# dog-qiuqiu/Yolo-FastestV2

Measured on AMD Instinct MI355X. Metric: images/sec at 352x352 bs=256 per GPU (forward+decode+NMS), higher is better.
Workload: dtype f32 tensors; contractions fp16x3 (two-term fp16 split operands on v_mfma_f32_16x16x32_f16, fp32 accumulate); depthwise/BN/ReLU/decode/NMS fp32 VALU; 1 GPU

## Files before the change

### include/yfv2.h

```cpp
#ifndef YFV2_H
#define YFV2_H

#include <stdint.h>

#ifdef __cplusplus
extern "C" {
#endif

#define YFV2_ABI_VERSION 7
#define YFV2_API __attribute__((visibility("default")))
#define YFV2_MAX_DET 300

typedef enum yfv2_status {
  YFV2_OK = 0,
  YFV2_ERR_ARG = -1,
  YFV2_ERR_CONFIG = -2,
  YFV2_ERR_DEVICE = -3,
  YFV2_ERR_WEIGHTS = -4,
  YFV2_ERR_STATE = -5,
  YFV2_ERR_BATCH = -6,
  YFV2_ERR_RANGE = -7
} yfv2_status;

typedef struct yfv2_ctx* yfv2_handle;
// ... 302 lines not shown
YFV2_API int32_t yfv2_num_rows(yfv2_handle h);
YFV2_API int32_t yfv2_num_stages(yfv2_handle h);

YFV2_API int yfv2_stage_info(yfv2_handle h, int32_t i, char* name, int32_t name_cap, double* flops_per_image,
                    double* bytes_per_image, double* external_bytes_per_image);
YFV2_API int yfv2_stage_kernel(yfv2_handle h, int32_t i, char* name, int32_t name_cap);

YFV2_API int yfv2_profile_forward(yfv2_handle h, const float* x, int32_t B, float* const out6[6], int32_t iters,
                         float* ms, void* stream);

YFV2_API int yfv2_clock_probe_begin(yfv2_handle h, int32_t workgroups, float milliseconds, int32_t busy, void* stream);
YFV2_API int yfv2_clock_probe_end(yfv2_handle h, double out[6], void* stream);

YFV2_API int yfv2_debug_repeat_step(yfv2_handle h, const float* x, int32_t B, float* const out6[6], int32_t step, int32_t iters, void* stream);

YFV2_API int yfv2_debug_post(yfv2_handle h, const float* const out6[6], int32_t B, float conf_thres, double iou_thres,
                             float* dets, int32_t* idx, int32_t* count, void* stream);

YFV2_API int64_t yfv2_debug_activation(yfv2_handle h, int32_t which, int32_t B, float* host_dst, int64_t cap);

YFV2_API int64_t yfv2_debug_train_relu_output(yfv2_handle h, const char* conv_name, float* host_dst, int64_t capacity);
YFV2_API int64_t yfv2_debug_train_tensor(yfv2_handle h, const char* name, int32_t which, float* host_dst, int64_t capacity);

YFV2_API int yfv2_debug_plan_dryrun(const yfv2_config* cfg, const yfv2_tensor_desc* tensors, int32_t n, int32_t* n_steps, int64_t* blob_floats);
YFV2_API int yfv2_debug_plan_dryrun_ex(const yfv2_config* cfg, const yfv2_plan* plan, const yfv2_tensor_desc* tensors, int32_t n, int32_t* n_steps,
                                       int64_t* blob_floats);
YFV2_API int64_t yfv2_debug_plan_image(const yfv2_config* cfg, const yfv2_tensor_desc* tensors, int32_t n, int32_t step, char* name,
                                       int32_t name_cap, float* dst, int64_t cap);
YFV2_API int64_t yfv2_debug_plan_image_ex(const yfv2_config* cfg, const yfv2_plan* plan, const yfv2_tensor_desc* tensors, int32_t n, int32_t step,
                                          char* name, int32_t name_cap, float* dst, int64_t cap);
YFV2_API int yfv2_debug_plan_c2_label(const yfv2_config* cfg, const yfv2_tensor_desc* tensors, int32_t n, int32_t* label);
YFV2_API int yfv2_debug_rows(int32_t row_kind, int32_t yuv, int32_t w, int32_t W, int64_t* lds_bytes, int32_t* max_width);
YFV2_API int yfv2_debug_rows16(int32_t row_kind, int32_t w, int32_t W, int64_t* lds_bytes, int32_t* max_width);

#ifdef __cplusplus
}
#endif
#endif
```

### yolo_fastestv2_amd/_lib.py

```python
import ctypes as C
import os

_HERE = os.path.dirname(os.path.abspath(__file__))
LIB_PATH = os.environ.get("YFV2_LIB") or os.path.join(_HERE, "libyfv2.so")
ABI_VERSION = 7
MAX_DET = 300

OK, ERR_ARG, ERR_CONFIG, ERR_DEVICE, ERR_WEIGHTS, ERR_STATE, ERR_BATCH, ERR_RANGE = 0, -1, -2, -3, -4, -5, -6, -7


class Config(C.Structure):
    _fields_ = [("classes", C.c_int32), ("anchor_num", C.c_int32), ("height", C.c_int32), ("width", C.c_int32),
                ("anchors", C.c_double * 12), ("max_batch", C.c_int32), ("device", C.c_int32)]


class Plan(C.Structure):
    _fields_ = [("struct_size", C.c_int32), ("fp32_matrix", C.c_int32), ("layer_by_layer", C.c_int32), ("post_two_launches", C.c_int32),
                ("front_two_launches", C.c_int32), ("towers_unpaired", C.c_int32), ("lanes", C.c_int32), ("trace", C.c_int32), ("trace_step", C.c_int32)]


PLAN_FIELDS = ("fp32_matrix", "layer_by_layer", "post_two_launches", "front_two_launches", "towers_unpaired", "lanes", "trace", "trace_step")


def make_plan(plan=None):
# ... 162 lines not shown
    "yfv2_track_update_motion": (C.c_int, [C.c_void_p, C.c_void_p, C.c_void_p, C.c_int32, C.c_int32, C.POINTER(C.c_int32), C.c_void_p, C.c_int32,
                                           C.POINTER(TrackRule), C.POINTER(TrackMotion), C.c_void_p, C.c_void_p, C.c_void_p, C.c_void_p, C.c_void_p,
                                           C.c_void_p, C.c_void_p]),
    "yfv2_track_update_two_pass": (C.c_int, [C.c_void_p, C.c_void_p, C.c_void_p, C.c_int32, C.c_int32, C.POINTER(C.c_int32), C.c_void_p, C.c_int32,
                                             C.POINTER(TrackRule), C.POINTER(TrackMotion), C.POINTER(TrackSecond), C.c_void_p, C.c_void_p, C.c_void_p,
                                             C.c_void_p, C.c_void_p, C.c_void_p, C.c_void_p, C.c_void_p]),
    "yfv2_track_feature_words": (C.c_int64, [C.c_int32, C.c_int32]),
    "yfv2_track_cosine": (C.c_int, [C.POINTER(C.c_float), C.POINTER(C.c_float), C.c_int32, C.POINTER(C.c_float), C.POINTER(C.c_float)]),
    "yfv2_track_feature_step": (C.c_int, [C.POINTER(C.c_float), C.c_int32, C.POINTER(C.c_float), C.c_int32, C.c_float, C.POINTER(C.c_float),
                                          C.POINTER(C.c_int32)]),
    "yfv2_track_update_appearance": (C.c_int, [C.c_void_p, C.c_void_p, C.c_void_p, C.c_int32, C.c_int32, C.POINTER(C.c_int32), C.c_void_p, C.c_int32,
                                               C.POINTER(TrackRule), C.POINTER(TrackMotion), C.POINTER(TrackSecond), C.POINTER(TrackAppearance),
                                               C.c_void_p, C.c_void_p, C.c_void_p, C.c_void_p, C.c_void_p, C.c_void_p, C.c_void_p, C.c_void_p,
                                               C.c_void_p, C.c_void_p, C.c_void_p]),
    "yfv2_export_maps": (C.c_int, [C.c_void_p, C.POINTER(C.c_void_p), C.c_int32, C.c_void_p, C.c_void_p, C.c_void_p]),
    "yfv2_deploy_post": (C.c_int, [C.c_void_p, C.c_void_p, C.c_void_p, C.c_int32, C.c_void_p, C.c_float, C.c_float, C.c_void_p, C.c_void_p,
                                   C.c_int32, C.c_void_p]),
    "yfv2_deploy_dropped": (C.c_int, [C.c_void_p, C.POINTER(C.c_int32), C.c_void_p]),
    "yfv2_detect_deploy_frames_u8": (C.c_int, [C.c_void_p, C.POINTER(Frame), C.c_int32, C.c_float, C.c_float, C.c_void_p, C.c_void_p,
                                               C.c_int32, C.c_void_p]),
    "yfv2_anchor_kmeans": (C.c_int, [C.c_void_p, C.c_void_p, C.c_int64, C.c_void_p, C.c_int32, C.c_int32, C.c_void_p, C.c_void_p,
                                     C.POINTER(KmeansInfo), C.c_void_p]),
    "yfv2_debug_kmeans_group": (C.c_int, [C.c_void_p, C.c_int32]),
    "yfv2_ap_per_class": (C.c_int, [C.c_void_p, C.c_void_p, C.c_void_p, C.c_void_p, C.c_int64, C.c_void_p, C.c_int64, C.POINTER(ApResult), C.c_void_p]),
    "yfv2_ap_per_class_multi": (C.c_int, [C.c_void_p, C.c_void_p, C.c_void_p, C.c_void_p, C.c_int64, C.c_void_p, C.c_int64, C.c_int32,
                                          C.POINTER(ApResult), C.c_void_p]),
    "yfv2_debug_plan_dryrun": (C.c_int, [C.c_void_p, C.c_void_p, C.c_int32, C.POINTER(C.c_int32), C.POINTER(C.c_int64)]),
    "yfv2_debug_plan_dryrun_ex": (C.c_int, [C.c_void_p, C.POINTER(Plan), C.c_void_p, C.c_int32, C.POINTER(C.c_int32), C.POINTER(C.c_int64)]),
    "yfv2_debug_plan_image": (C.c_int64, [C.c_void_p, C.c_void_p, C.c_int32, C.c_int32, C.c_char_p, C.c_int32, C.c_void_p, C.c_int64]),
    "yfv2_debug_plan_image_ex": (C.c_int64, [C.c_void_p, C.POINTER(Plan), C.c_void_p, C.c_int32, C.c_int32, C.c_char_p, C.c_int32, C.c_void_p, C.c_int64]),
    "yfv2_debug_plan_c2_label": (C.c_int, [C.c_void_p, C.c_void_p, C.c_int32, C.POINTER(C.c_int32)]),
    "yfv2_debug_rows": (C.c_int, [C.c_int32, C.c_int32, C.c_int32, C.c_int32, C.POINTER(C.c_int64), C.POINTER(C.c_int32)]),
    "yfv2_debug_rows16": (C.c_int, [C.c_int32, C.c_int32, C.c_int32, C.POINTER(C.c_int64), C.POINTER(C.c_int32)]),
    "yfv2_num_rows": (C.c_int32, [C.c_void_p]),
    "yfv2_num_stages": (C.c_int32, [C.c_void_p]),
    "yfv2_stage_info": (C.c_int, [C.c_void_p, C.c_int32, C.c_char_p, C.c_int32, C.POINTER(C.c_double),
                                  C.POINTER(C.c_double), C.POINTER(C.c_double)]),
    "yfv2_stage_kernel": (C.c_int, [C.c_void_p, C.c_int32, C.c_char_p, C.c_int32]),
    "yfv2_profile_forward": (C.c_int, [C.c_void_p, C.c_void_p, C.c_int32, C.POINTER(C.c_void_p), C.c_int32,
                                       C.POINTER(C.c_float), C.c_void_p]),
    "yfv2_debug_repeat_step": (C.c_int, [C.c_void_p, C.c_void_p, C.c_int32, C.POINTER(C.c_void_p), C.c_int32, C.c_int32, C.c_void_p]),
    "yfv2_debug_post": (C.c_int, [C.c_void_p, C.POINTER(C.c_void_p), C.c_int32, C.c_float, C.c_double, C.c_void_p, C.c_void_p,
                                  C.c_void_p, C.c_void_p]),
    "yfv2_debug_activation": (C.c_int64, [C.c_void_p, C.c_int32, C.c_int32, C.c_void_p, C.c_int64]),
    "yfv2_debug_train_relu_output": (C.c_int64, [C.c_void_p, C.c_char_p, C.c_void_p, C.c_int64]),
    "yfv2_debug_train_tensor": (C.c_int64, [C.c_void_p, C.c_char_p, C.c_int32, C.c_void_p, C.c_int64]),
}

_lib = None


def lib():
    global _lib
    if _lib is not None:
        return _lib
    if not os.path.exists(LIB_PATH):
        raise ImportError("%s is missing: the HIP extension has not been built (run __graft_entry__.build()); "
                          "yolo_fastestv2_amd has no CPU or PyTorch fallback" % LIB_PATH)
    L = C.CDLL(LIB_PATH)
    if not hasattr(L, "yfv2_abi_version"):
        raise ImportError("%s does not export yfv2_abi_version: not a libyfv2 build" % LIB_PATH)
    L.yfv2_abi_version.restype, L.yfv2_abi_version.argtypes = C.c_int, []
    if L.yfv2_abi_version() != ABI_VERSION:
        raise ImportError("libyfv2.so ABI %d != binding ABI %d: rebuild (__graft_entry__.build())" % (L.yfv2_abi_version(), ABI_VERSION))
    for name, (res, args) in _PROTOTYPES.items():
        if name.startswith("yfv2_debug_") and os.environ.get("YFV2_LIB") and not hasattr(L, name):
# ... 17 lines not shown
```

### yolo_fastestv2_amd/csrc/yfv2_api_debug.hip

```cpp
#include <algorithm>
#include <cstdio>
#include <variant>

#include "yfv2_ctx.h"

namespace {

struct DryRun {
  yfv2_ctx ctx;
  WeightPacker wp;
  int build(const yfv2_config* cfg, const yfv2_plan* plan, const yfv2_tensor_desc* tensors, int32_t n) {
    int rows = 0;
    if (int rc = check_config(cfg, &rows)) return rc;
    uintptr_t next = 0x100000000ull;
    auto fake = [&](yfv2_ctx* hh, Buf* b, size_t per_img) {
      b->per_img = per_img;
      b->p = reinterpret_cast<float*>(next);
      next += (per_img * sizeof(float) * (size_t)hh->cfg.max_batch + 4095) & ~(uintptr_t)4095;
      return (int)YFV2_OK;
    };
    setup_ctx(&ctx, cfg, rows, fake);
    read_plan_switches(&ctx, plan);
    return build_plan(&ctx, wp, tensors, n, nullptr);
  }
// ... 41 lines not shown
  const size_t img = job >= 0 ? tw->halves[job].img : step_image(view[step]);
  if (name && name_cap > 0) std::snprintf(name, (size_t)name_cap, "%s", st_name.c_str());
  const int64_t avail = (int64_t)d.wp.blob.size() - (int64_t)img;
  const int64_t cnt = avail < cap ? avail : cap;
  if (cnt > 0) std::memcpy(dst, &d.wp.blob[img], sizeof(float) * (size_t)cnt);
  return cnt;
}

int yfv2_debug_plan_c2_label(const yfv2_config* cfg, const yfv2_tensor_desc* tensors, int32_t n, int32_t* label) {
  if (!cfg || !tensors || n <= 0 || !label) return fail(nullptr, YFV2_ERR_ARG, "yfv2_debug_plan_c2_label: bad argument");
  DryRun d;
  if (int rc = d.build(cfg, nullptr, tensors, n)) return rc;
  for (int k = 0; k < 96; ++k) label[k] = d.ctx.plan.c2_permuted ? d.ctx.plan.c2_label[k] : k;
  return d.ctx.plan.c2_permuted ? 1 : 0;
}

int yfv2_debug_rows(int32_t row_kind, int32_t yuv, int32_t w, int32_t W, int64_t* lds_bytes, int32_t* max_width) {
  if (row_kind < 0 || row_kind >= YFV2_ROW_KINDS || yuv < 0 || yuv > 1 || w < 1 || w > (1 << 26) || W < 1 || W > (1 << 20))
    return fail(nullptr, YFV2_ERR_ARG, "yfv2_debug_rows: bad argument");
  const Yfv2FrameKind frames = yuv ? YFV2_FRAMES_YUV8 : YFV2_FRAMES_BGR;
  if (lds_bytes) *lds_bytes = (int64_t)yfv2_rows_lds_bytes((Yfv2RowKind)row_kind, frames, w, W);
  if (max_width) *max_width = yfv2_rows_max_width((Yfv2RowKind)row_kind, frames, W);
  return YFV2_OK;
}

int yfv2_debug_rows16(int32_t row_kind, int32_t w, int32_t W, int64_t* lds_bytes, int32_t* max_width) {
  if (row_kind < 0 || row_kind >= YFV2_ROW_KINDS || w < 1 || w > (1 << 26) || W < 1 || W > (1 << 20))
    return fail(nullptr, YFV2_ERR_ARG, "yfv2_debug_rows16: bad argument");
  if (lds_bytes) *lds_bytes = (int64_t)yfv2_rows_lds_bytes((Yfv2RowKind)row_kind, YFV2_FRAMES_YUV16, w, W);
  if (max_width) *max_width = yfv2_rows_max_width((Yfv2RowKind)row_kind, YFV2_FRAMES_YUV16, W);
  return YFV2_OK;
}

int yfv2_clock_probe_begin(yfv2_handle h, int32_t workgroups, float milliseconds, int32_t busy, void* stream) {
  if (!h || workgroups < 1 || workgroups > 4096 || !(milliseconds > 0.f) || milliseconds > 10000.f)
    return fail(h, YFV2_ERR_ARG, "yfv2_clock_probe_begin: bad argument");
  DeviceGuard guard(h->device);
  if (!h->d_probe) HIP_TRY(h, hipMalloc(reinterpret_cast<void**>(&h->d_probe), 4096 * 4 * sizeof(unsigned long long)));
  int khz = 0;
  if (hipDeviceGetAttribute(&khz, hipDeviceAttributeWallClockRate, h->device) != hipSuccess || khz <= 0) khz = 100000;
  ClockProbeArgs a{};
  a.out = h->d_probe; a.busy = busy ? 1 : 0;
  a.ref_ticks = (unsigned long long)((double)milliseconds * (double)khz);
  h->probe_wgs = workgroups;
  if (!yfv2_launch_clock_probe(a, workgroups, static_cast<hipStream_t>(stream))) return fail(h, YFV2_ERR_DEVICE, "clock probe launch failed");
  return YFV2_OK;
}

int yfv2_clock_probe_end(yfv2_handle h, double out[6], void* stream) {
  if (!h || !out) return fail(h, YFV2_ERR_ARG, "yfv2_clock_probe_end: null argument");
  if (!h->d_probe || h->probe_wgs < 1) return fail(h, YFV2_ERR_STATE, "yfv2_clock_probe_end without yfv2_clock_probe_begin");
  DeviceGuard guard(h->device);
  hipStream_t s = static_cast<hipStream_t>(stream);
  std::vector<unsigned long long> st((size_t)h->probe_wgs * 4);
  HIP_TRY(h, hipMemcpyAsync(st.data(), h->d_probe, st.size() * sizeof(unsigned long long), hipMemcpyDeviceToHost, s));
  HIP_TRY(h, hipStreamSynchronize(s));
  int khz = 0;
  if (hipDeviceGetAttribute(&khz, hipDeviceAttributeWallClockRate, h->device) != hipSuccess || khz <= 0) khz = 100000;
  const double ref_mhz = khz * 1e-3;
  double mn = 1e30, mx = 0., sum = 0., ms = 0.;
  unsigned xcds = 0;
  for (int i = 0; i < h->probe_wgs; ++i) {
    const double cyc = (double)st[4 * i], ref = (double)st[4 * i + 1];
    if (!(ref > 0.)) return fail(h, YFV2_ERR_DEVICE, "clock probe: a workgroup reported no reference ticks");
    const double mhz = cyc / ref * ref_mhz;
    mn = std::min(mn, mhz); mx = std::max(mx, mhz); sum += mhz; ms += ref / ref_mhz * 1e-3;
// ... 155 lines not shown
```

### yolo_fastestv2_amd/csrc/yfv2_block.hip

```cpp
#include <cstdlib>
#include <type_traits>

#include "yfv2_device.h"

template <int C2>
struct S1Cfg {
  static constexpr int KC = (C2 + 15) / 16;
  static constexpr int DW_FL = 9 * KC * 16;
  static constexpr int CST_FL = 6 * KC * 16;
};

constexpr int CH_TBL_FL = 64;

constexpr int CH6_WP_FL = 3 * 3 * 256;
constexpr int CH6_IMG_FL = 2 * CH6_WP_FL + S1Cfg<48>::DW_FL + S1Cfg<48>::CST_FL + CH_TBL_FL;

__host__ __device__ constexpr int s1chain_pitch(int PW) { return 2 * (PW + 1) + ((PW - 2 * (PW + 1)) % 16 + 16) % 16; }
__host__ __device__ constexpr int s1chain_plane(int PH, int PW) { return (2 * (PH + 1) * s1chain_pitch(PW) + 15) & ~15; }

template <int THREADS>
__global__ __launch_bounds__(THREADS, 2) void block_s1chain6_kernel(BlockS1Args a) {
  constexpr int C2 = 48;
  using Cfg = S1Cfg<C2>;
  constexpr int KC = Cfg::KC, NQ = C2 / 4, C = 2 * C2, NT = 4;
  constexpr int NW = THREADS / 64;
  constexpr int N4 = CH6_IMG_FL / 4, NIT = (N4 + THREADS - 1) / THREADS;
  extern __shared__ __attribute__((aligned(16))) float lds[];
  float* IM = lds;
  float* T1 = lds + CH6_IMG_FL;
  const float* W1P = IM;
  const float* W2P = IM + CH6_WP_FL;
  const float* WD = IM + 2 * CH6_WP_FL;
  const float* CS = WD + Cfg::DW_FL;
  const int H = a.H, W = a.W, HW = H * W, NB = a.nblk;
// ... 322 lines not shown
  const long pl = s1chain_plane(H / 2, W / 2);
  return (long)CH6_IMG_FL + 12L * pl * 4;
}

long yfv2_s1chain_park_floats(int H, int W, int nblk) { return 12L * (nblk - 2) * ((((H / 2) * (W / 2) + 15) & ~15) * 4); }

int yfv2_s1chain_image_floats() { return CH6_IMG_FL; }

bool yfv2_s1chain_supported(int c2, int H, int W) {
  if (c2 != 48 || H < 2 || (H & 1) || (W & 1)) return false;
  if ((H / 2) * (W / 2) > 16 * 8) return false;
  if (yfv2_s1chain_park_floats(H, W, 7) > 24L * (4 * H) * (4 * W)) return false;
  return s1chain_lds_floats(H, W) * 4 <= YFV2_LDS_FULL;
}

bool yfv2_launch_block_s1chain(const BlockS1Args& a, hipStream_t s) {
  if (!yfv2_s1chain_supported(48, a.H, a.W) || a.nblk < 2) return false;
  const size_t lds = sizeof(float) * (size_t)s1chain_lds_floats(a.H, a.W);
  const Yfv2Device dev = yfv2_device();
  YFV2_LAUNCH_LDS(dev, (block_s1chain6_kernel<512>), YFV2_LDS_FULL, dim3(yfv2_image_grid(a.B, dev)), dim3(512), lds, s, a);
  return true;
}

constexpr int P96_C2 = 96, P96_C = 192, P96_KC = 6, P96_TH = 3, P96_TC = 32;
constexpr int P96_CPP = P96_C + 4;
constexpr int P96_TP = P96_TC + 4;
constexpr int P96_W1_FL = 2 * P96_KC * 256, P96_W2_FL = P96_KC * 2 * 256;
constexpr int P96_IMG_FL = P96_W1_FL + P96_W2_FL + 9 * P96_TC + 4 * P96_TC + 2 * P96_C2;
constexpr int P96_W1P_FL = 2 * (P96_KC / 2) * 2 * 256, P96_W2P_FL = P96_KC * 1 * 2 * 256;
constexpr int P96_IMGP_FL = P96_W1P_FL + P96_W2P_FL + 9 * P96_TC + 4 * P96_TC + 2 * P96_C2;
constexpr int P96_MAXPX = 128;

template <int THREADS, bool PRE>
__global__ __launch_bounds__(THREADS, 2) void block_s1pool_kernel(BlockS1Args a) {
  constexpr int NW = THREADS / 64;
  constexpr int IMG_FL = PRE ? P96_IMGP_FL : P96_IMG_FL;
  constexpr int W1_FL = PRE ? P96_W1P_FL : P96_W1_FL, W2_FL = PRE ? P96_W2P_FL : P96_W2_FL;
  constexpr int N4 = IMG_FL / 4, NIT = (N4 + THREADS - 1) / THREADS;
  extern __shared__ __attribute__((aligned(16))) float lds[];
  float* POOL = lds;
  float* T = POOL + a.H * a.W * P96_CPP;
  float* IMG = T + (a.H + 2) * (a.W + 2) * P96_TP;
  Yfv2Watch watch;
  const int H = a.H, W = a.W, HW = H * W, WP = W + 2, NB = a.nblk;
  const float invW = 1.0f / (float)W;
  const int tid = threadIdx.x, lane = tid & 63, p = lane & 15, g = lane >> 4, wave = tid >> 6;
  const int px = 16 * wave + p;
  const bool pv = px < HW;
  const int pxc = pv ? px : HW - 1;
  const int py = yfv2_fdiv(pxc, invW), pxx = pxc - py * W;
  float* tpix = T + ((py + 1) * WP + pxx + 1) * P96_TP;
  const float* twin = T + (py * WP + pxx) * P96_TP;
  float* ppix = POOL + pxc * P96_CPP;
  static_assert(NW * 16 >= P96_MAXPX, "one tile per wave");

  YFV2_WSTAMP(0);
  for (int i = tid; i < (H + 2) * WP * P96_TP / 4; i += THREADS) reinterpret_cast<f32x4*>(T)[i] = (f32x4){0.f, 0.f, 0.f, 0.f};

  for (int b = blockIdx.x; b < a.B; b += gridDim.x) {
    {
      const f32x4* src = reinterpret_cast<const f32x4*>(a.in + (size_t)b * HW * P96_C);
      const f32x4* isrc = reinterpret_cast<const f32x4*>(a.img);
      constexpr int NPX = (P96_MAXPX * (P96_C / 4) + THREADS - 1) / THREADS;
      const int n4 = HW * (P96_C / 4);
      f32x4 ti[NIT];
#pragma unroll
      for (int k = 0; k < NIT; ++k) { const int i = tid + k * THREADS; ti[k] = i < N4 ? isrc[i] : (f32x4){0.f, 0.f, 0.f, 0.f}; }
#pragma unroll
      for (int k0 = 0; k0 < NPX; k0 += 6) {
        f32x4 tp[6];
#pragma unroll
        for (int k = 0; k < 6; ++k) { const int i = tid + (k0 + k) * THREADS; tp[k] = i < n4 ? src[i] : (f32x4){0.f, 0.f, 0.f, 0.f}; }
#pragma unroll
        for (int k = 0; k < 6; ++k) {
          const int i = tid + (k0 + k) * THREADS;
          const int ipx = i / (P96_C / 4), q = i - ipx * (P96_C / 4);
          if (i < n4) *reinterpret_cast<f32x4*>(POOL + ipx * P96_CPP + 4 * q) = tp[k];
        }
      }
#pragma unroll
      for (int k = 0; k < NIT; ++k) { const int i = tid + k * THREADS; if (i < N4) reinterpret_cast<f32x4*>(IMG)[i] = ti[k]; }
    }
    __syncthreads();
    YFV2_WSTAMP(1);

#pragma unroll 1
    for (int blk = 0; blk < NB; ++blk) {
      f32x4 acc2[P96_KC];
#pragma unroll
      for (int mt = 0; mt < P96_KC; ++mt) acc2[mt] = (f32x4){0.f, 0.f, 0.f, 0.f};
      yfv2_h8 b1a[PRE ? P96_KC / 2 : 1], b1b[PRE ? P96_KC / 2 : 1];
      auto split_pair = [&](f32x4 c0, f32x4 c1, yfv2_h8& t1, yfv2_h8& t2) __attribute__((always_inline)) {
        u32x4 u1, u2;
        const f32x4 cs[2] = {c0 * 16.0f, c1 * 16.0f};
#pragma unroll
        for (int e = 0; e < 2; ++e) {
          const u32x4 t = split_f16x2(cs[e]);
          u1[2 * e] = t[0]; u1[2 * e + 1] = t[1]; u2[2 * e] = t[2]; u2[2 * e + 1] = t[3];
        }
        t1 = __builtin_bit_cast(yfv2_h8, u1); t2 = __builtin_bit_cast(yfv2_h8, u2);
      };
      if constexpr (PRE) {
#pragma unroll
        for (int sp = 0; sp < P96_KC / 2; ++sp) {
          f32x4 c[2];
#pragma unroll
          for (int e = 0; e < 2; ++e) {
            const int s2 = 2 * sp + e;
            const f32x4 q0 = *reinterpret_cast<const f32x4*>(ppix + 32 * s2 + 8 * g);
            const f32x4 q1 = *reinterpret_cast<const f32x4*>(ppix + 32 * s2 + 8 * g + 4);
            c[e] = (f32x4){q0[1], q0[3], q1[1], q1[3]};
          }
          split_pair(c[0], c[1], b1a[sp], b1b[sp]);
        }
      }
#pragma unroll 1
      for (int th = 0; th < P96_TH; ++th) {
        const int t = blk * P96_TH + th;
        const bool more = t + 1 < NB * P96_TH;
        const float* W1t = IMG;
        const float* W2t = IMG + W1_FL;
        const float* TAPS = W2t + W2_FL;
        const float* CSV = TAPS + 9 * P96_TC;
        f32x4 nimg[NIT];
        {
          const f32x4* isrc = reinterpret_cast<const f32x4*>(a.img + (size_t)(t + 1) * IMG_FL);
#pragma unroll
          for (int k = 0; k < NIT; ++k) { const int i = tid + k * THREADS; nimg[k] = (more && i < N4) ? isrc[i] : (f32x4){0.f, 0.f, 0.f, 0.f}; }
        }
        {
          f32x4 acc1[2] = {{0.f, 0.f, 0.f, 0.f}, {0.f, 0.f, 0.f, 0.f}};
          if constexpr (PRE) {
#pragma unroll
            for (int sp = 0; sp < P96_KC / 2; ++sp) {
              yfv2_h8 a1[2], a2[2];
#pragma unroll
              for (int mt = 0; mt < 2; ++mt) {
                const float* wq2 = W1t + (((mt * (P96_KC / 2) + sp) * 2) * 64 + lane) * 4;
                a1[mt] = __builtin_bit_cast(yfv2_h8, *reinterpret_cast<const u32x4*>(wq2));
                a2[mt] = __builtin_bit_cast(yfv2_h8, *reinterpret_cast<const u32x4*>(wq2 + 256));
              }
#define P96_PROD(A_, B_) _Pragma("unroll") for (int mt = 0; mt < 2; ++mt) acc1[mt] = __builtin_amdgcn_mfma_f32_16x16x32_f16(A_[mt], B_, acc1[mt], 0, 0, 0);
              P96_PROD(a1, b1b[sp]) P96_PROD(a2, b1a[sp]) P96_PROD(a1, b1a[sp])
#undef P96_PROD
            }
            watch.see(acc1[0][0]);
          } else {
#pragma unroll
          for (int s2 = 0; s2 < P96_KC; ++s2) {
            const f32x4 q0 = *reinterpret_cast<const f32x4*>(ppix + 32 * s2 + 8 * g);
            const f32x4 q1 = *reinterpret_cast<const f32x4*>(ppix + 32 * s2 + 8 * g + 4);
            const f32x4 bf = {q0[1], q0[3], q1[1], q1[3]};
            const f32x4 a0 = *reinterpret_cast<const f32x4*>(W1t + ((0 * P96_KC + s2) * 64 + lane) * 4);
            const f32x4 a1 = *reinterpret_cast<const f32x4*>(W1t + ((1 * P96_KC + s2) * 64 + lane) * 4);
#pragma unroll
            for (int j = 0; j < 4; ++j) {
              acc1[0] = __builtin_amdgcn_mfma_f32_16x16x4f32(a0[j], bf[j], acc1[0], 0, 0, 0);
              acc1[1] = __builtin_amdgcn_mfma_f32_16x16x4f32(a1[j], bf[j], acc1[1], 0, 0, 0);
            }
          }
          }
          if (pv) {
#pragma unroll
            for (int mt = 0; mt < 2; ++mt) {
              const f32x4 sc = *reinterpret_cast<const f32x4*>(CSV + 0 * P96_TC + 16 * mt + 4 * g);
              const f32x4 sh = *reinterpret_cast<const f32x4*>(CSV + 1 * P96_TC + 16 * mt + 4 * g);
              f32x4 y;
#pragma unroll
              for (int c = 0; c < 4; ++c) { const float u = __builtin_fmaf(acc1[mt][c], sc[c], sh[c]); y[c] = u > 0.f ? u : 0.f; }
              *reinterpret_cast<f32x4*>(tpix + 16 * mt + 4 * g) = y;
            }
          }
        }
        if (blk == 0) YFV2_WSTAMP(2 + 4 * th);
        __syncthreads();
        if (blk == 0) YFV2_WSTAMP(3 + 4 * th);
        if constexpr (PRE) {
          f32x4 bfr2[2];
#pragma unroll
          for (int c2 = 0; c2 < 2; ++c2) {
            const int cb = 16 * c2 + 4 * g;
            f32x4 win[9], wl[9];
#pragma unroll
            for (int k = 0; k < 9; ++k) {
              win[k] = *reinterpret_cast<const f32x4*>(twin + ((k / 3) * WP + (k % 3)) * P96_TP + cb);
// ... 19 lines not shown
            a2[mt] = __builtin_bit_cast(yfv2_h8, *reinterpret_cast<const u32x4*>(wq2 + 256));
          }
#define P96_PROD(A_, B_) _Pragma("unroll") for (int mt = 0; mt < P96_KC; ++mt) acc2[mt] = __builtin_amdgcn_mfma_f32_16x16x32_f16(A_[mt], B_, acc2[mt], 0, 0, 0);
          P96_PROD(a1, x2) P96_PROD(a2, x1) P96_PROD(a1, x1)
#undef P96_PROD
        } else {
#pragma unroll
        for (int c2 = 0; c2 < 2; ++c2) {
          const int cb = 16 * c2 + 4 * g;
          f32x4 win[9], wl[9], af[P96_KC];
#pragma unroll
          for (int k = 0; k < 9; ++k) {
            win[k] = *reinterpret_cast<const f32x4*>(twin + ((k / 3) * WP + (k % 3)) * P96_TP + cb);
            wl[k] = *reinterpret_cast<const f32x4*>(TAPS + k * P96_TC + cb);
          }
          const f32x4 dsc = *reinterpret_cast<const f32x4*>(CSV + 2 * P96_TC + cb);
          const f32x4 dsh = *reinterpret_cast<const f32x4*>(CSV + 3 * P96_TC + cb);
#pragma unroll
          for (int mt = 0; mt < P96_KC; ++mt) af[mt] = *reinterpret_cast<const f32x4*>(W2t + ((mt * 2 + c2) * 64 + lane) * 4);
          __builtin_amdgcn_sched_barrier(0);
          f32x4 d = {0.f, 0.f, 0.f, 0.f}, bfr;
#pragma unroll
          for (int k = 0; k < 9; ++k)
#pragma unroll
            for (int c = 0; c < 4; ++c) d[c] = __builtin_fmaf(win[k][c], wl[k][c], d[c]);
#pragma unroll
          for (int c = 0; c < 4; ++c) bfr[c] = __builtin_fmaf(d[c], dsc[c], dsh[c]);
#pragma unroll
          for (int j = 0; j < 4; ++j)
#pragma unroll
            for (int mt = 0; mt < P96_KC; ++mt) acc2[mt] = __builtin_amdgcn_mfma_f32_16x16x4f32(af[mt][j], bfr[j], acc2[mt], 0, 0, 0);
        }
        }
        if (th == P96_TH - 1) {
          if constexpr (PRE) watch.see(acc2[0][0]);
#pragma unroll
          for (int mt = 0; mt < P96_KC; ++mt) {
            const f32x4 sc = *reinterpret_cast<const f32x4*>(CSV + 4 * P96_TC + 16 * mt + 4 * g);
            const f32x4 sh = *reinterpret_cast<const f32x4*>(CSV + 4 * P96_TC + P96_C2 + 16 * mt + 4 * g);
#pragma unroll
            for (int c = 0; c < 4; ++c) { const float u = __builtin_fmaf(acc2[mt][c], sc[c], sh[c]); acc2[mt][c] = u > 0.f ? u : 0.f; }
          }
        }
        if (blk == 0) YFV2_WSTAMP(4 + 4 * th);
        __syncthreads();
        if (more) {
#pragma unroll
          for (int k = 0; k < NIT; ++k) { const int i = tid + k * THREADS; if (i < N4) reinterpret_cast<f32x4*>(IMG)[i] = nimg[k]; }
        }
        if (th < P96_TH - 1) __syncthreads();
        if (blk == 0) YFV2_WSTAMP(5 + 4 * th);
      }
      {
        constexpr int NQ = P96_C2 / 4;
        constexpr int NEV = (P96_MAXPX * NQ + THREADS - 1) / THREADS;
        f32x4 ev[NEV];
#pragma unroll
        for (int k = 0; k < NEV; ++k) {
          const int i = tid + k * THREADS;
          const int ipx = i / NQ, q = i - ipx * NQ;
          ev[k] = (f32x4){0.f, 0.f, 0.f, 0.f};
          if (ipx < HW) {
            const f32x4 q0 = *reinterpret_cast<const f32x4*>(POOL + ipx * P96_CPP + 8 * q);
            const f32x4 q1 = *reinterpret_cast<const f32x4*>(POOL + ipx * P96_CPP + 8 * q + 4);
            ev[k] = (f32x4){q0[0], q0[2], q1[0], q1[2]};
          }
        }
        __syncthreads();
#pragma unroll
        for (int k = 0; k < NEV; ++k) {
          const int i = tid + k * THREADS;
          const int ipx = i / NQ, q = i - ipx * NQ;
          if (ipx < HW) *reinterpret_cast<f32x4*>(POOL + ipx * P96_CPP + 4 * q) = ev[k];
        }
        if (pv) {
#pragma unroll
          for (int mt = 0; mt < P96_KC; ++mt) *reinterpret_cast<f32x4*>(ppix + P96_C2 + 16 * mt + 4 * g) = acc2[mt];
        }
        __syncthreads();
        YFV2_WSTAMP(14 + blk);
      }
    }
    {
      f32x4* dst = reinterpret_cast<f32x4*>(a.out + (size_t)b * HW * P96_C);
      for (int i = tid; i < HW * (P96_C / 4); i += THREADS) {
        const int ipx = i / (P96_C / 4), q = i - ipx * (P96_C / 4);
        dst[i] = *reinterpret_cast<const f32x4*>(POOL + ipx * P96_CPP + 4 * q);
      }
    }
    YFV2_WSTAMP(17);
    __syncthreads();
  }
  watch.report(a.nonfinite);
}

static long s1pool_lds_floats(int H, int W, bool pre) { return (long)H * W * P96_CPP + (long)(H + 2) * (W + 2) * P96_TP + (pre ? P96_IMGP_FL : P96_IMG_FL); }
int yfv2_s1pool_image_floats(bool presplit) { return presplit ? P96_IMGP_FL : P96_IMG_FL; }
bool yfv2_s1pool_supported(int c2, int H, int W) {
  if (c2 != P96_C2 || H * W > P96_MAXPX || H * W < 1) return false;
  return s1pool_lds_floats(H, W, true) * 4 <= YFV2_LDS_FULL;
}

bool yfv2_launch_block_s1pool(const BlockS1Args& a, hipStream_t s) {
  if (!yfv2_s1pool_supported(P96_C2, a.H, a.W) || a.nblk < 1) return false;
  const size_t lds = sizeof(float) * (size_t)s1pool_lds_floats(a.H, a.W, a.presplit != 0);
  const Yfv2Device dev = yfv2_device();
  const int blocks = yfv2_image_grid(a.B, dev);
  if (a.presplit) YFV2_LAUNCH_LDS(dev, (block_s1pool_kernel<512, true>), YFV2_LDS_FULL, dim3(blocks), dim3(512), lds, s, a);
  else YFV2_LAUNCH_LDS(dev, (block_s1pool_kernel<512, false>), YFV2_LDS_FULL, dim3(blocks), dim3(512), lds, s, a);
  return true;
}

constexpr int TW_C = 72, TW_KC = 5;
constexpr int TW_WP_FL = TW_KC * TW_KC * 256;
constexpr int TW_WH_FL = TW_KC * 256;

template <int CIN>
struct S2Cfg {
  static constexpr int KC = (CIN + 15) / 16;
  static constexpr int CP = CIN + 4;
  static constexpr int W_FL = KC * KC * 256;
  static constexpr int DW_FL = 9 * KC * 16;
  static constexpr int NCS = 10;
  static constexpr int MAXP = 14;
  static constexpr int MAXT = CIN <= 24 ? 10 : 6;
};

template <int CIN, int THREADS, bool PPIN>
__global__ __launch_bounds__(THREADS) void block_s2_kernel(BlockS2Args a) {
  using Cfg = S2Cfg<CIN>;
  constexpr int KC = Cfg::KC, CP = Cfg::CP, KS = KC * 16;
  constexpr int NW = THREADS / 64;
  constexpr int CO = 2 * CIN;
  extern __shared__ __attribute__((aligned(16))) float lds[];
  float* W1 = lds;
  float* W2 = W1 + Cfg::W_FL;
  float* WJ = W2 + Cfg::W_FL;
  float* WD = WJ + Cfg::W_FL;
  float* WE = WD + Cfg::DW_FL;
  float* CS = WE + Cfg::DW_FL;
  float* T1 = CS + Cfg::NCS * KS;
  const int H = a.H, W = a.W, R = a.R, OH = H >> 1, OW = W >> 1;
// ... 894 lines not shown
```

### yolo_fastestv2_amd/csrc/yfv2_internal.h

```cpp
#pragma once
#include <hip/hip_runtime.h>
#include <hip/hip_ext.h>
#include <stdint.h>

#include <atomic>

struct Yfv2LaunchProbe { hipEvent_t start = nullptr, stop = nullptr; int launches = 0; };
extern thread_local Yfv2LaunchProbe yfv2_launch_probe;
#define YFV2_LAUNCH(kernel, grid, block, lds, stream, ...)                                                                        \
  do {                                                                                                                             \
    Yfv2LaunchProbe& yfv2_lp_ = yfv2_launch_probe;                                                                                 \
    hipExtLaunchKernelGGL(kernel, grid, block, lds, stream, yfv2_lp_.launches++ == 0 ? yfv2_lp_.start : nullptr, yfv2_lp_.stop, 0, \
                          __VA_ARGS__);                                                                                            \
  } while (0)
struct Yfv2Device { int index, cus; };
inline Yfv2Device yfv2_device() {
  static std::atomic<int> cus_of[64];
  int dev = 0;
  if (hipGetDevice(&dev) != hipSuccess || dev < 0 || dev > 63) dev = 0;
  int cus = cus_of[dev].load(std::memory_order_relaxed);
  if (cus <= 0) { if (hipDeviceGetAttribute(&cus, hipDeviceAttributeMultiprocessorCount, dev) != hipSuccess || cus <= 0) cus = 256; cus_of[dev].store(cus, std::memory_order_relaxed); }
  return {dev, cus};
}
inline int yfv2_device_cus() { return yfv2_device().cus; }
// ... 56 lines not shown
struct DwArgs {
  const float* in;
  float* out;
  const float* w;
  const float* scale;
  const float* shift;
  int B, H, W, C;
  int OH, OW;
  int in_stride, in_off;
  int out_stride, out_off;
  int relu;
};

struct BlockS1Args {
  const float* in;
  float* out;
  const float* img;
  long long* trace;
  int B, H, W;
  int R;
  int nblk;
  int presplit;
  int* nonfinite;
  float* park;
};

bool yfv2_s1chain_supported(int c2, int H, int W);
int yfv2_s1chain_image_floats();
long yfv2_s1chain_park_floats(int H, int W, int nblk);
bool yfv2_launch_block_s1chain(const BlockS1Args& a, hipStream_t s);
bool yfv2_s1pool_supported(int c2, int H, int W);
int yfv2_s1pool_image_floats(bool presplit);
bool yfv2_launch_block_s1pool(const BlockS1Args& a, hipStream_t s);

struct BlockS2Args {
  const float* in;
  float* out;
  const float* img;
  int B, H, W;
  int R;
  int s4_main_bands;
  int pp_in;
  unsigned pp_mask;
  long long pp_bufstride;
  long long pp_imgstride;
  int bf6;
  long long* trace;
  const float* img16;
  int* nonfinite;
};
bool yfv2_s3h_supported(int H, int W);
void yfv2_launch_s3h(const BlockS2Args& a, hipStream_t s);
bool yfv2_s4h_supported(int H, int W);
void yfv2_launch_s4h(const BlockS2Args& a, hipStream_t s);

__host__ __device__ inline int yfv2_stage2_channel(int slot) {
  const int p = slot >> 1, e = slot & 1;
  const int b0 = p / 12, b1 = (p % 12) / 6, b2 = (p % 6) / 3, h = 2 * (p % 3) + e;
  return b0 + 2 * b1 + 4 * b2 + 8 * h;
}
struct S1PxArgs {
  float* act;
  const float* img;
  int B, H, W;
  int nstrips, nb, R;
  int img_stride;
// ... 419 lines not shown
```

Measured before the change: 478,200 images/s.

## Replace per-block channel shuffle in s1pool kernel with host-planned LDS slot tables

Precomputes, on the host, a channel-to-LDS-slot assignment for the stride-1 ShuffleNet block chain so the channel shuffle between blocks becomes pure addressing. The in-kernel gather/scatter pass that repacked even channels after every block, along with its two barriers, is removed. Loads, stores and operand reads now go through small byte tables passed as a kernel argument and copied into LDS. The next-tile weight prefetch store is split into two parts so one barrier per tile can be dropped. This adds table lookups, some scalar and two-element stores, and extra LDS for the table.

```diff
diff --git a/include/yfv2.h b/include/yfv2.h
--- a/include/yfv2.h
+++ b/include/yfv2.h
@@ -358,6 +358,7 @@
 YFV2_API int yfv2_debug_plan_c2_label(const yfv2_config* cfg, const yfv2_tensor_desc* tensors, int32_t n, int32_t* label);
 YFV2_API int yfv2_debug_rows(int32_t row_kind, int32_t yuv, int32_t w, int32_t W, int64_t* lds_bytes, int32_t* max_width);
 YFV2_API int yfv2_debug_rows16(int32_t row_kind, int32_t w, int32_t W, int64_t* lds_bytes, int32_t* max_width);
+YFV2_API int64_t yfv2_debug_s1pool_slots(int32_t nblk, void* dst, int64_t cap);
 
 #ifdef __cplusplus
 }
diff --git a/yolo_fastestv2_amd/_lib.py b/yolo_fastestv2_amd/_lib.py
--- a/yolo_fastestv2_amd/_lib.py
+++ b/yolo_fastestv2_amd/_lib.py
@@ -218,6 +218,7 @@
     "yfv2_debug_plan_c2_label": (C.c_int, [C.c_void_p, C.c_void_p, C.c_int32, C.POINTER(C.c_int32)]),
     "yfv2_debug_rows": (C.c_int, [C.c_int32, C.c_int32, C.c_int32, C.c_int32, C.POINTER(C.c_int64), C.POINTER(C.c_int32)]),
     "yfv2_debug_rows16": (C.c_int, [C.c_int32, C.c_int32, C.c_int32, C.POINTER(C.c_int64), C.POINTER(C.c_int32)]),
+    "yfv2_debug_s1pool_slots": (C.c_int64, [C.c_int32, C.c_void_p, C.c_int64]),
     "yfv2_num_rows": (C.c_int32, [C.c_void_p]),
     "yfv2_num_stages": (C.c_int32, [C.c_void_p]),
     "yfv2_stage_info": (C.c_int, [C.c_void_p, C.c_int32, C.c_char_p, C.c_int32, C.POINTER(C.c_double),
diff --git a/yolo_fastestv2_amd/csrc/yfv2_api_debug.hip b/yolo_fastestv2_amd/csrc/yfv2_api_debug.hip
--- a/yolo_fastestv2_amd/csrc/yfv2_api_debug.hip
+++ b/yolo_fastestv2_amd/csrc/yfv2_api_debug.hip
@@ -97,6 +97,13 @@
   return YFV2_OK;
 }
 
+int64_t yfv2_debug_s1pool_slots(int32_t nblk, void* dst, int64_t cap) {
+  S1PoolSlots t;
+  if (!dst || cap < (int64_t)sizeof(t) || !yfv2_s1pool_slots(nblk, &t)) return fail(nullptr, YFV2_ERR_ARG, "yfv2_debug_s1pool_slots: bad argument");
+  std::memcpy(dst, &t, sizeof(t));
+  return (int64_t)sizeof(t);
+}
+
 int yfv2_clock_probe_begin(yfv2_handle h, int32_t workgroups, float milliseconds, int32_t busy, void* stream) {
   if (!h || workgroups < 1 || workgroups > 4096 || !(milliseconds > 0.f) || milliseconds > 10000.f)
     return fail(h, YFV2_ERR_ARG, "yfv2_clock_probe_begin: bad argument");
diff --git a/yolo_fastestv2_amd/csrc/yfv2_block.hip b/yolo_fastestv2_amd/csrc/yfv2_block.hip
--- a/yolo_fastestv2_amd/csrc/yfv2_block.hip
+++ b/yolo_fastestv2_amd/csrc/yfv2_block.hip
@@ -1,5 +1,8 @@
 #include <cstdlib>
+#include <cstring>
+#include <numeric>
 #include <type_traits>
+#include <vector>
 
 #include "yfv2_device.h"
 
@@ -388,15 +391,21 @@
 constexpr int P96_MAXPX = 128;
 
 template <int THREADS, bool PRE>
-__global__ __launch_bounds__(THREADS, 2) void block_s1pool_kernel(BlockS1Args a) {
+__global__ __launch_bounds__(THREADS, 2) void block_s1pool_kernel(BlockS1Args a, S1PoolSlots sl) {
   constexpr int NW = THREADS / 64;
   constexpr int IMG_FL = PRE ? P96_IMGP_FL : P96_IMG_FL;
   constexpr int W1_FL = PRE ? P96_W1P_FL : P96_W1_FL, W2_FL = PRE ? P96_W2P_FL : P96_W2_FL;
   constexpr int N4 = IMG_FL / 4, NIT = (N4 + THREADS - 1) / THREADS;
+  constexpr int QW1 = W1_FL / 4, QMID = (W2_FL + 9 * P96_TC) / 4, QS1 = 2 * P96_TC / 4;
+  constexpr int N4A = QW1 + QS1, N4B = N4 - N4A;
+  constexpr int NITA = (N4A + THREADS - 1) / THREADS, NITB = (N4B + THREADS - 1) / THREADS;
+  auto quad_a = [](int j) { return j < QW1 ? j : QMID + j; };
+  auto quad_b = [](int j) { return j < QMID ? QW1 + j : QS1 + QW1 + j; };
   extern __shared__ __attribute__((aligned(16))) float lds[];
   float* POOL = lds;
   float* T = POOL + a.H * a.W * P96_CPP;
   float* IMG = T + (a.H + 2) * (a.W + 2) * P96_TP;
+  unsigned* TBL = reinterpret_cast<unsigned*>(IMG + IMG_FL);
   Yfv2Watch watch;
   const int H = a.H, W = a.W, HW = H * W, WP = W + 2, NB = a.nblk;
   const float invW = 1.0f / (float)W;
@@ -412,12 +421,33 @@
 
   YFV2_WSTAMP(0);
   for (int i = tid; i < (H + 2) * WP * P96_TP / 4; i += THREADS) reinterpret_cast<f32x4*>(T)[i] = (f32x4){0.f, 0.f, 0.f, 0.f};
+  constexpr int TBL_W = sizeof(sl.lane) / 4;
+  if (tid < TBL_W) TBL[tid] = (&sl.lane[0][0][0])[tid];
+  static_assert(3 * THREADS % (P96_C / 4) == 0, "a thread's quads repeat with period 3");
+  unsigned rec[3];
+#pragma unroll
+  for (int m = 0; m < 3; ++m) rec[m] = sl.io[(tid + m * THREADS) % (P96_C / 4)];
+  auto put_quad = [](float* pix, unsigned rc, int r, f32x4 v) __attribute__((always_inline)) {
+    const unsigned o0 = rc & 255u, o1 = (rc >> 8) & 255u, o2 = (rc >> 16) & 255u;
+    if (r == 0) {
+      *reinterpret_cast<f32x4*>(pix + o0) = v;
+    } else {
+      *reinterpret_cast<f32x2*>(pix + o1) = (f32x2){v[1], v[3]};
+      if (r == 1) {
+        *reinterpret_cast<f32x2*>(pix + o0) = (f32x2){v[0], v[2]};
+      } else {
+        pix[o0] = v[0];
+        pix[o2] = v[2];
+      }
+    }
+  };
 
   for (int b = blockIdx.x; b < a.B; b += gridDim.x) {
     {
       const f32x4* src = reinterpret_cast<const f32x4*>(a.in + (size_t)b * HW * P96_C);
       const f32x4* isrc = reinterpret_cast<const f32x4*>(a.img);
       constexpr int NPX = (P96_MAXPX * (P96_C / 4) + THREADS - 1) / THREADS;
+      static_assert(NPX % 6 == 0, "two batches of six");
       const int n4 = HW * (P96_C / 4);
       f32x4 ti[NIT];
 #pragma unroll
@@ -430,8 +460,8 @@
 #pragma unroll
         for (int k = 0; k < 6; ++k) {
           const int i = tid + (k0 + k) * THREADS;
-          const int ipx = i / (P96_C / 4), q = i - ipx * (P96_C / 4);
-          if (i < n4) *reinterpret_cast<f32x4*>(POOL + ipx * P96_CPP + 4 * q) = tp[k];
+          const int ipx = i / (P96_C / 4);
+          if (i < n4) put_quad(POOL + ipx * P96_CPP, rec[(k0 + k) % 3], NB, tp[k]);
         }
       }
 #pragma unroll
@@ -456,19 +486,14 @@
         }
         t1 = __builtin_bit_cast(yfv2_h8, u1); t2 = __builtin_bit_cast(yfv2_h8, u2);
       };
+      const unsigned* ltab = TBL + (blk * 4 + g) * 8;
+      const u32x2 rdw = *reinterpret_cast<const u32x2*>(ltab + 6);
+      auto operand_quad = [&](int s2) __attribute__((always_inline)) {
+        return *reinterpret_cast<const f32x4*>(ppix + ((rdw[s2 >> 2] >> (8 * (s2 & 3))) & 255u));
+      };
       if constexpr (PRE) {
 #pragma unroll
-        for (int sp = 0; sp < P96_KC / 2; ++sp) {
-          f32x4 c[2];
-#pragma unroll
-          for (int e = 0; e < 2; ++e) {
-            const int s2 = 2 * sp + e;
-            const f32x4 q0 = *reinterpret_cast<const f32x4*>(ppix + 32 * s2 + 8 * g);
-            const f32x4 q1 = *reinterpret_cast<const f32x4*>(ppix + 32 * s2 + 8 * g + 4);
-            c[e] = (f32x4){q0[1], q0[3], q1[1], q1[3]};
-          }
-          split_pair(c[0], c[1], b1a[sp], b1b[sp]);
-        }
+        for (int sp = 0; sp < P96_KC / 2; ++sp) split_pair(operand_quad(2 * sp), operand_quad(2 * sp + 1), b1a[sp], b1b[sp]);
       }
 #pragma unroll 1
       for (int th = 0; th < P96_TH; ++th) {
@@ -478,11 +503,13 @@
         const float* W2t = IMG + W1_FL;
         const float* TAPS = W2t + W2_FL;
         const float* CSV = TAPS + 9 * P96_TC;
-        f32x4 nimg[NIT];
+        f32x4 nia[NITA], nib[NITB];
         {
           const f32x4* isrc = reinterpret_cast<const f32x4*>(a.img + (size_t)(t + 1) * IMG_FL);
 #pragma unroll
-          for (int k = 0; k < NIT; ++k) { const int i = tid + k * THREADS; nimg[k] = (more && i < N4) ? isrc[i] : (f32x4){0.f, 0.f, 0.f, 0.f}; }
+          for (int k = 0; k < NITA; ++k) { const int j = tid + k * THREADS; nia[k] = (more && j < N4A) ? isrc[quad_a(j)] : (f32x4){0.f, 0.f, 0.f, 0.f}; }
+#pragma unroll
+          for (int k = 0; k < NITB; ++k) { const int j = tid + k * THREADS; nib[k] = (more && j < N4B) ? isrc[quad_b(j)] : (f32x4){0.f, 0.f, 0.f, 0.f}; }
         }
         {
           f32x4 acc1[2] = {{0.f, 0.f, 0.f, 0.f}, {0.f, 0.f, 0.f, 0.f}};
@@ -504,9 +531,7 @@
           } else {
 #pragma unroll
           for (int s2 = 0; s2 < P96_KC; ++s2) {
-            const f32x4 q0 = *reinterpret_cast<const f32x4*>(ppix + 32 * s2 + 8 * g);
-            const f32x4 q1 = *reinterpret_cast<const f32x4*>(ppix + 32 * s2 + 8 * g + 4);
-            const f32x4 bf = {q0[1], q0[3], q1[1], q1[3]};
+            const f32x4 bf = operand_quad(s2);
             const f32x4 a0 = *reinterpret_cast<const f32x4*>(W1t + ((0 * P96_KC + s2) * 64 + lane) * 4);
             const f32x4 a1 = *reinterpret_cast<const f32x4*>(W1t + ((1 * P96_KC + s2) * 64 + lane) * 4);
 #pragma unroll
@@ -592,6 +617,10 @@
             for (int mt = 0; mt < P96_KC; ++mt) acc2[mt] = __builtin_amdgcn_mfma_f32_16x16x4f32(af[mt][j], bfr[j], acc2[mt], 0, 0, 0);
         }
         }
+        if (more) {
+#pragma unroll
+          for (int k = 0; k < NITA; ++k) { const int j = tid + k * THREADS; if (j < N4A) reinterpret_cast<f32x4*>(IMG)[quad_a(j)] = nia[k]; }
+        }
         if (th == P96_TH - 1) {
           if constexpr (PRE) watch.see(acc2[0][0]);
 #pragma unroll
@@ -601,51 +630,34 @@
 #pragma unroll
             for (int c = 0; c < 4; ++c) { const float u = __builtin_fmaf(acc2[mt][c], sc[c], sh[c]); acc2[mt][c] = u > 0.f ? u : 0.f; }
           }
+          if (pv) {
+            const u32x4 f0 = *reinterpret_cast<const u32x4*>(ltab);
+            const unsigned f1 = ltab[4];
+            auto tb = [&](int i) __attribute__((always_inline)) { return ((i < 16 ? f0[i >> 2] : f1) >> (8 * (i & 3))) & 255u; };
+#pragma unroll
+            for (int mt = 0; mt < P96_KC; ++mt)
+              put_quad(ppix, tb(3 * mt) | (tb(3 * mt + 1) << 8) | (tb(3 * mt + 2) << 16), NB - 1 - blk, acc2[mt]);
+          }
         }
         if (blk == 0) YFV2_WSTAMP(4 + 4 * th);
         __syncthreads();
         if (more) {
 #pragma unroll
-          for (int k = 0; k < NIT; ++k) { const int i = tid + k * THREADS; if (i < N4) reinterpret_cast<f32x4*>(IMG)[i] = nimg[k]; }
-        }
-        if (th < P96_TH - 1) __syncthreads();
+          for (int k = 0; k < NITB; ++k) { const int j = tid + k * THREADS; if (j < N4B) reinterpret_cast<f32x4*>(IMG)[quad_b(j)] = nib[k]; }
+        }
         if (blk == 0) YFV2_WSTAMP(5 + 4 * th);
       }
-      {
-        constexpr int NQ = P96_C2 / 4;
-        constexpr int NEV = (P96_MAXPX * NQ + THREADS - 1) / THREADS;
-        f32x4 ev[NEV];
-#pragma unroll
-        for (int k = 0; k < NEV; ++k) {
-          const int i = tid + k * THREADS;
-          const int ipx = i / NQ, q = i - ipx * NQ;
-          ev[k] = (f32x4){0.f, 0.f, 0.f, 0.f};
-          if (ipx < HW) {
-            const f32x4 q0 = *reinterpret_cast<const f32x4*>(POOL + ipx * P96_CPP + 8 * q);
-            const f32x4 q1 = *reinterpret_cast<const f32x4*>(POOL + ipx * P96_CPP + 8 * q + 4);
-            ev[k] = (f32x4){q0[0], q0[2], q1[0], q1[2]};
-          }
-        }
-        __syncthreads();
-#pragma unroll
-        for (int k = 0; k < NEV; ++k) {
-          const int i = tid + k * THREADS;
-          const int ipx = i / NQ, q = i - ipx * NQ;
-          if (ipx < HW) *reinterpret_cast<f32x4*>(POOL + ipx * P96_CPP + 4 * q) = ev[k];
-        }
-        if (pv) {
-#pragma unroll
-          for (int mt = 0; mt < P96_KC; ++mt) *reinterpret_cast<f32x4*>(ppix + P96_C2 + 16 * mt + 4 * g) = acc2[mt];
-        }
-        __syncthreads();
-        YFV2_WSTAMP(14 + blk);
-      }
+      YFV2_WSTAMP(14 + blk);
     }
     {
       f32x4* dst = reinterpret_cast<f32x4*>(a.out + (size_t)b * HW * P96_C);
-      for (int i = tid; i < HW * (P96_C / 4); i += THREADS) {
-        const int ipx = i / (P96_C / 4), q = i - ipx * (P96_C / 4);
-        dst[i] = *reinterpret_cast<const f32x4*>(POOL + ipx * P96_CPP + 4 * q);
+      constexpr int NPX = (P96_MAXPX * (P96_C / 4) + THREADS - 1) / THREADS;
+      const int n4 = HW * (P96_C / 4);
+#pragma unroll
+      for (int k = 0; k < NPX; ++k) {
+        const int i = tid + k * THREADS;
+        const int ipx = i / (P96_C / 4);
+        if (i < n4) dst[i] = *reinterpret_cast<const f32x4*>(POOL + ipx * P96_CPP + (rec[k % 3] >> 24));
       }
     }
     YFV2_WSTAMP(17);
@@ -654,7 +666,86 @@
   watch.report(a.nonfinite);
 }
 
-static long s1pool_lds_floats(int H, int W, bool pre) { return (long)H * W * P96_CPP + (long)(H + 2) * (W + 2) * P96_TP + (pre ? P96_IMGP_FL : P96_IMG_FL); }
+bool yfv2_s1pool_slots(int nblk, S1PoolSlots* t) {
+  if (nblk < 1 || nblk > S1POOL_MAX_BLOCKS || !t) return false;
+  std::memset(t, 0, sizeof(*t));
+  constexpr int NQ = P96_C / 4, NOP = P96_C2 / 4;
+  const int nch = P96_C + P96_C2 * nblk, nrq = NOP * nblk + NQ;
+  std::vector<int> cur(P96_C), quad_of(nch, -1), elem_of(nch, -1), origin(nrq, -1), slot(nrq, -1);
+  std::iota(cur.begin(), cur.end(), 0);
+  auto origin_of = [](int id) { return id < P96_C ? 0 : 1 + (id - P96_C) / P96_C2; };
+  auto claim = [&](int rq, int e, int id) {
+    if (quad_of[id] != -1 || (e > 0 && origin[rq] != origin_of(id))) return false;
+    quad_of[id] = rq, elem_of[id] = e, origin[rq] = origin_of(id);
+    return true;
+  };
+  for (int k = 0; k < nblk; ++k) {
+    for (int qi = 0; qi < NOP; ++qi)
+      for (int e = 0; e < 4; ++e)
+        if (!claim(NOP * k + qi, e, cur[8 * qi + 2 * e + 1])) return false;
+    std::vector<int> nxt(P96_C);
+    for (int i = 0; i < P96_C2; ++i) nxt[i] = cur[2 * i], nxt[P96_C2 + i] = P96_C + P96_C2 * k + i;
+    cur = nxt;
+  }
+  for (int q = 0; q < NQ; ++q)
+    for (int e = 0; e < 4; ++e)
+      if (!claim(NOP * nblk + q, e, cur[4 * q + e])) return false;
+  for (int o = 0; o <= nblk; ++o) {
+    std::vector<int> avail;
+    for (int i = 0; i < (o == 0 ? NQ : NOP); ++i) avail.push_back(o == 0 ? i : slot[NOP * (o - 1) + i]);
+    auto take = [&](int res) {
+      size_t at = 0;
+      for (size_t i = 0; i < avail.size(); ++i)
+        if (avail[i] % 16 == res) { at = i; break; }
+      const int s = avail[at];
+      avail.erase(avail.begin() + (long)at);
+      return s;
+    };
+    for (int rq = 0; rq < nrq; ++rq) {
+      if (origin[rq] != o) continue;
+      if (avail.empty()) return false;
+      int res = -1;
+      if (rq < NOP * nblk) {
+        const int mate = rq ^ 1;
+        if (slot[mate] >= 0) res = slot[mate] % 16;
+        else if (origin[mate] == o)
+          for (size_t i = 0; i < avail.size() && res < 0; ++i)
+            for (size_t j = i + 1; j < avail.size() && res < 0; ++j)
+              if (avail[i] % 16 == avail[j] % 16) res = avail[i] % 16;
+      }
+      slot[rq] = take(res);
+    }
+    if (!avail.empty()) return false;
+  }
+  auto off = [&](int id) { return 4 * slot[quad_of[id]] + elem_of[id]; };
+  auto pieces = [&](int id, int r, unsigned* rec) {
+    const int o0 = off(id), o1 = off(id + 1), o2 = off(id + 2), o3 = off(id + 3);
+    if (r == 0 ? (o0 % 4 != 0 || o1 != o0 + 1 || o2 != o0 + 2 || o3 != o0 + 3) : (o1 % 2 != 0 || o3 != o1 + 1)) return false;
+    if (r == 1 && (o0 % 2 != 0 || o2 != o0 + 1)) return false;
+    *rec = (unsigned)o0 | (unsigned)o1 << 8 | (unsigned)o2 << 16;
+    return true;
+  };
+  auto set_byte = [](unsigned* words, int i, int v) { words[i >> 2] |= (unsigned)v << (8 * (i & 3)); };
+  for (int z = 0; z < NQ; ++z) {
+    if (!pieces(4 * z, nblk, &t->io[z])) return false;
+    set_byte(&t->io[z], 3, 4 * slot[NOP * nblk + z]);
+  }
+  for (int k = 0; k < nblk; ++k)
+    for (int g = 0; g < 4; ++g) {
+      unsigned* rec = t->lane[k][g];
+      for (int mt = 0; mt < P96_KC; ++mt) {
+        unsigned pc = 0;
+        if (!pieces(P96_C + P96_C2 * k + 4 * (4 * mt + g), nblk - 1 - k, &pc)) return false;
+        for (int j = 0; j < 3; ++j) set_byte(rec, 3 * mt + j, (int)(pc >> (8 * j)) & 255);
+      }
+      for (int s2 = 0; s2 < P96_KC; ++s2) set_byte(rec, 24 + s2, 4 * slot[NOP * k + 4 * s2 + g]);
+    }
+  return true;
+}
+
+static long s1pool_lds_floats(int H, int W, bool pre) {
+  return (long)H * W * P96_CPP + (long)(H + 2) * (W + 2) * P96_TP + (pre ? P96_IMGP_FL : P96_IMG_FL) + (long)(sizeof(S1PoolSlots::lane) / 4);
+}
 int yfv2_s1pool_image_floats(bool presplit) { return presplit ? P96_IMGP_FL : P96_IMG_FL; }
 bool yfv2_s1pool_supported(int c2, int H, int W) {
   if (c2 != P96_C2 || H * W > P96_MAXPX || H * W < 1) return false;
@@ -662,12 +753,20 @@
 }
 
 bool yfv2_launch_block_s1pool(const BlockS1Args& a, hipStream_t s) {
-  if (!yfv2_s1pool_supported(P96_C2, a.H, a.W) || a.nblk < 1) return false;
+  if (!yfv2_s1pool_supported(P96_C2, a.H, a.W) || a.nblk < 1 || a.nblk > S1POOL_MAX_BLOCKS) return false;
+  struct Tables { S1PoolSlots t[S1POOL_MAX_BLOCKS]; bool ok[S1POOL_MAX_BLOCKS]; };
+  static const Tables tables = [] {
+    Tables r;
+    for (int n = 1; n <= S1POOL_MAX_BLOCKS; ++n) r.ok[n - 1] = yfv2_s1pool_slots(n, &r.t[n - 1]);
+    return r;
+  }();
+  if (!tables.ok[a.nblk - 1]) return false;
+  const S1PoolSlots& sl = tables.t[a.nblk - 1];
   const size_t lds = sizeof(float) * (size_t)s1pool_lds_floats(a.H, a.W, a.presplit != 0);
   const Yfv2Device dev = yfv2_device();
   const int blocks = yfv2_image_grid(a.B, dev);
-  if (a.presplit) YFV2_LAUNCH_LDS(dev, (block_s1pool_kernel<512, true>), YFV2_LDS_FULL, dim3(blocks), dim3(512), lds, s, a);
-  else YFV2_LAUNCH_LDS(dev, (block_s1pool_kernel<512, false>), YFV2_LDS_FULL, dim3(blocks), dim3(512), lds, s, a);
+  if (a.presplit) YFV2_LAUNCH_LDS(dev, (block_s1pool_kernel<512, true>), YFV2_LDS_FULL, dim3(blocks), dim3(512), lds, s, a, sl);
+  else YFV2_LAUNCH_LDS(dev, (block_s1pool_kernel<512, false>), YFV2_LDS_FULL, dim3(blocks), dim3(512), lds, s, a, sl);
   return true;
 }
 
diff --git a/yolo_fastestv2_amd/csrc/yfv2_internal.h b/yolo_fastestv2_amd/csrc/yfv2_internal.h
--- a/yolo_fastestv2_amd/csrc/yfv2_internal.h
+++ b/yolo_fastestv2_amd/csrc/yfv2_internal.h
@@ -112,6 +112,12 @@
 bool yfv2_s1pool_supported(int c2, int H, int W);
 int yfv2_s1pool_image_floats(bool presplit);
 bool yfv2_launch_block_s1pool(const BlockS1Args& a, hipStream_t s);
+constexpr int S1POOL_MAX_BLOCKS = 3;
+struct S1PoolSlots {
+  unsigned io[48];
+  unsigned lane[S1POOL_MAX_BLOCKS][4][8];
+};
+bool yfv2_s1pool_slots(int nblk, S1PoolSlots* t);
 
 struct BlockS2Args {
   const float* in;
```

Result: no change. 478,000 images/s (-0.0%).
